# wwyuan2023/VITS

Measured on AMD Instinct MI355X. Metric: 22.05 kHz audio samples/sec/GPU (infer RTF) + train utt/sec at 1/2/4/8 MI355X, higher is better.
Workload: dtype fp32; 1 GPU; SynthesizerTrn.infer_p2 batch=16 Tx=100 Ty=500 (configs/base.json, 16 kHz, hop 192) per GPU; global_batch=16, seq_len=500, parallelism=single GPU, graph=False

## Files before the change

vits_amd/csrc/resblock_f32p.hip:

```cpp
#include "conv1d_impl.h"

namespace {

using vits_conv::fast_sigmoid;
using vits_conv::fast_tanh;
using vits_conv::split3_bf16x4;

constexpr int RP_GROUP = 3;
struct RpGroup {
  vits_resblock_pair_desc d[RP_GROUP];
  int n;
  int batch;
};

typedef __bf16 bf16x8 __attribute__((ext_vector_type(8)));
typedef __bf16 bf16x4 __attribute__((ext_vector_type(4)));
typedef __bf16 bf16x2 __attribute__((ext_vector_type(2)));
typedef float f32x4v __attribute__((ext_vector_type(4)));

template <int MODE>
struct RpT {
  typedef float xt;
  typedef __bf16 lt;
  static constexpr int NPL = 3;
};
template <>
struct RpT<1> {
  typedef __bf16 xt;
  typedef __bf16 lt;
  static constexpr int NPL = 1;
};
template <>
struct RpT<2> {
  typedef _Float16 xt;
  typedef _Float16 lt;
  static constexpr int NPL = 1;
};
__host__ __device__ constexpr int rp_npl(int mode) { return mode == 0 ? 3 : 1; }

__host__ __device__ constexpr int rp_ng(int C) { return C <= 64 ? 256 : 128; }
__host__ __device__ constexpr int rp_threads(int C) { return C == 256 ? 512 : 256; }
__host__ __device__ constexpr int rp_kc(int C, int mode = 0) {
  return C == 256 ? 64 : 16;
}
__host__ __device__ inline int rp_xcols(int NG, int k, int dil) {
  return ((NG + (k - 1) * dil + 3 + 3) >> 2) << 2;
}
__host__ __device__ inline int rp_lds_bytes(int C, int k, int dil, int mode = 0) {
  const int NG = rp_ng(C), npl = rp_npl(mode);
  const int xs = 2 * npl * rp_xcols(NG, k, dil) * (rp_kc(C, mode) + 4);
  const int gsz = npl * (NG + 16) * (C / 2 + 8);
  return 4 * 2 * C + 2 * (xs > gsz ? xs : gsz) + 64;
}
__host__ __device__ constexpr int rp_occ(int C, int) { return C == 256 ? 1 : 2; }

template <int C, int MODE = 0>
__global__ __launch_bounds__(rp_threads(C), rp_occ(C, MODE)) void resblock_f32p_kernel(
    const RpGroup G) {
  typedef typename RpT<MODE>::xt xt;
  typedef typename RpT<MODE>::lt lt;
  constexpr int NPL = RpT<MODE>::NPL;
  typedef lt lt8 __attribute__((ext_vector_type(8)));
  typedef lt lt4 __attribute__((ext_vector_type(4)));
  typedef lt lt2 __attribute__((ext_vector_type(2)));
  typedef xt xt4 __attribute__((ext_vector_type(4)));
  constexpr int H = C / 2;
  constexpr int NT = rp_threads(C);
  constexpr int WAVES_M = C >= 64 ? C / 64 : 1;
  constexpr int WAVES_N = NT / 64 / WAVES_M;
  constexpr int NG = 64 * WAVES_N;
  static_assert(NG == rp_ng(C), "tile columns");
  constexpr int TM = C >= 64 ? 2 : 1, TN = 2;
  constexpr int KC = rp_kc(C, MODE);
  constexpr int KCP = KC + 4;
  constexpr int GP = H + 8;
  constexpr int GPL = (NG + 16) * GP;
  constexpr int S1 = C / 16, S2 = H / 16;
  constexpr int NU = ((KC / 4) * ((NG + 102) / 4) + NT - 1) / NT;
  typedef lt8 av_t;
  constexpr int NB = NPL == 3 ? TN : 1;

  const int gi = (int)blockIdx.z / G.batch;
  const int b = (int)blockIdx.z - gi * G.batch;
  const vits_resblock_pair_desc& p = G.d[gi];
  const int Tn = p.t_len;
  const int L = p.lengths ? min(Tn, (int)p.lengths[b]) : Tn;
  const int k = p.k;
  const int dil = p.dil;
  const int BN = NG - (k - 1);
  const int n0 = blockIdx.x * BN;
  if (n0 >= Tn) return;
  if (p.lengths && p.len_skip > 0 && n0 >= L + p.len_skip) return;

  extern __shared__ float smem[];
  float* const erow = smem;
  lt* const reg = reinterpret_cast<lt*>(smem + 2 * C);

  const int tid = threadIdx.x;
  const int lane = tid & 63;
  const int wid = tid >> 6;
  const int wn = (wid % WAVES_N) * 64;
  const int wm = (wid / WAVES_N) * 64;
  const int l32 = lane & 31;
  const int lhi = lane >> 5;
  const int p1 = (k - 1) * dil / 2;
  const int p2 = (k - 1) / 2;

  {
    const float* cond = p.cond ? p.cond + (int64_t)b * p.cond_bstride : nullptr;
    for (int r = tid; r < 2 * C; r += NT) {
      float e = 0.f;
      if (r < C) {
        const int idx = (r & 1) ? H + (r >> 1) : (r >> 1);
        if (p.b1) e = p.b1[idx];
        if (cond) e += cond[idx];
      } else if (p.b2) {
        e = p.b2[r - C];
      }
      erow[r] = e;
    }
  }

  f32x16 acc[TM][TN];
#pragma unroll
  for (int i = 0; i < TM; ++i)
#pragma unroll
    for (int j = 0; j < TN; ++j)
#pragma unroll
      for (int r = 0; r < 16; ++r) acc[i][j][r] = 0.f;

  auto mma = [&](av_t (*a)[TM], const av_t* bh, const av_t* bm, const av_t* bl) {
#pragma unroll
    for (int mi = 0; mi < TM; ++mi)
#pragma unroll
      for (int ni = 0; ni < TN; ++ni) {
        f32x16 c = acc[mi][ni];
        if constexpr (MODE == 0) {
          c = __builtin_amdgcn_mfma_f32_32x32x16_bf16(a[0][mi], bl[ni], c, 0, 0, 0);
          c = __builtin_amdgcn_mfma_f32_32x32x16_bf16(a[2][mi], bh[ni], c, 0, 0, 0);
          c = __builtin_amdgcn_mfma_f32_32x32x16_bf16(a[1][mi], bm[ni], c, 0, 0, 0);
          c = __builtin_amdgcn_mfma_f32_32x32x16_bf16(a[0][mi], bm[ni], c, 0, 0, 0);
          c = __builtin_amdgcn_mfma_f32_32x32x16_bf16(a[1][mi], bh[ni], c, 0, 0, 0);
          c = __builtin_amdgcn_mfma_f32_32x32x16_bf16(a[0][mi], bh[ni], c, 0, 0, 0);
        } else if constexpr (MODE == 1) {
          c = __builtin_amdgcn_mfma_f32_32x32x16_bf16(a[0][mi], bh[ni], c, 0, 0, 0);
        } else {
          c = __builtin_amdgcn_mfma_f32_32x32x16_f16(a[0][mi], bh[ni], c, 0, 0, 0);
        }
        acc[mi][ni] = c;
      }
  };
  auto loadA = [&](const lt* wl, int64_t wstep, int m_pad, int s, int total,
                   av_t (*a)[TM]) {
    const lt* wp = wl + (int64_t)(s < total ? s : total - 1) * wstep;
#pragma unroll
    for (int q = 0; q < NPL; ++q)
#pragma unroll
      for (int mi = 0; mi < TM; ++mi)
        a[q][mi] = *reinterpret_cast<const av_t*>(wp + ((int64_t)q * m_pad + mi * 32) * 8);
  };

  av_t a0[NPL][TM], a1[NPL][TM];
  av_t bh0[TN], bm0[NB], bl0[NB], bh1[TN], bm1[NB], bl1[NB];

  const xt* xb = reinterpret_cast<const xt*>(p.x) + (int64_t)b * p.x_bstride;
  {
    const int tw0 = n0 - p2 - p1;
    const int xstart = tw0 & ~3;
    const int xsh = tw0 - xstart;
    const int xcols = rp_xcols(NG, k, dil);
    const int nunits = (KC / 4) * (xcols >> 2);
    const int xpl = xcols * KCP;
    lt* const xbuf0 = reg;
    lt* const xbuf1 = reg + NPL * xpl;
    const float slope = p.in_slope;
    xt4 xr[NU][4];
    int xoff[NU];
    bool xok[NU];
#pragma unroll
    for (int q = 0; q < NU; ++q) {
      const int u = tid + NT * q;
      const int tt = xstart + 4 * (u / (KC / 4));
      xok[q] = u < nunits && tt >= 0 && tt < Tn;
      xoff[q] = xok[q] ? 4 * (u % (KC / 4)) * p.x_cstride + tt : 0;
    }
    auto gload = [&](int ch) {
      const xt* base = xb + (int64_t)ch * KC * p.x_cstride;
#pragma unroll
      for (int q = 0; q < NU; ++q) {
        if (q * NT < nunits) {
#pragma unroll
          for (int i = 0; i < 4; ++i) {
            const xt* src = xok[q] ? base + xoff[q] + i * p.x_cstride : xb;
            xr[q][i] = *reinterpret_cast<const xt4*>(src);
          }
        }
      }
    };
    auto lstore = [&](lt* xs) {
#pragma unroll
      for (int q = 0; q < NU; ++q) {
        const int u = tid + NT * q;
        if (q * NT < nunits && u < nunits) {
          f32x4v v[4];
#pragma unroll
          for (int i = 0; i < 4; ++i)
#pragma unroll
            for (int e = 0; e < 4; ++e) {
              float t = (float)xr[q][i][e];
              t = t < 0.f ? t * slope : t;
              v[i][e] = xok[q] ? t : 0.f;
            }
          lt* xh = xs + 4 * (u / (KC / 4)) * KCP + 4 * (u % (KC / 4));
#pragma unroll
          for (int e = 0; e < 4; ++e) {
            const f32x4v w = {v[0][e], v[1][e], v[2][e], v[3][e]};
            if constexpr (NPL == 3) {
              bf16x4 h4, m4, l4;
              split3_bf16x4(w, h4, m4, l4);
              *reinterpret_cast<bf16x4*>(xh + e * KCP) = h4;
              *reinterpret_cast<bf16x4*>(xh + xpl + e * KCP) = m4;
              *reinterpret_cast<bf16x4*>(xh + 2 * xpl + e * KCP) = l4;
            } else {
              lt4 w4;
#pragma unroll
              for (int i = 0; i < 4; ++i) w4[i] = (lt)w[i];
              *reinterpret_cast<lt4*>(xh + e * KCP) = w4;
            }
          }
        }
      }
    };
    auto loadB = [&](const lt* xs, int j, int g, av_t* bh, av_t* bm, av_t* bl) {
      const int P4 = xpl / 4;
#pragma unroll
      for (int ni = 0; ni < TN; ++ni) {
        const lt4* xp = reinterpret_cast<const lt4*>(
            xs + (wn + ni * 32 + l32 + j * dil + xsh) * KCP + 16 * g + 8 * lhi);
        bh[ni] = __builtin_shufflevector(xp[0], xp[1], 0, 1, 2, 3, 4, 5, 6, 7);
        if constexpr (NPL == 3) {
          bm[ni] = __builtin_shufflevector(xp[P4], xp[P4 + 1], 0, 1, 2, 3, 4, 5, 6, 7);
          bl[ni] = __builtin_shufflevector(xp[2 * P4], xp[2 * P4 + 1], 0, 1, 2, 3, 4, 5, 6, 7);
        }
      }
    };
    const lt* wl = reinterpret_cast<const lt*>(p.w1) +
                   ((int64_t)(lhi * NPL) * p.m_pad1 + wm + l32) * 8;
    const int64_t wstep = (int64_t)16 * NPL * p.m_pad1;
    const int total = S1 * k;
    const int nst = (KC / 16) * k;
    loadA(wl, wstep, p.m_pad1, 0, total, a0);
    gload(0);
    lstore(xbuf0);
    __syncthreads();
    for (int ch = 0; ch < C / KC; ++ch) {
      const bool more = ch + 1 < C / KC;
      if (more) gload(ch + 1);
      const lt* xs = (ch & 1) ? xbuf1 : xbuf0;
      const int s0 = ch * nst;
      int j = 0, g = 0;
      auto next = [&]() {
        if (++j == k) {
          j = 0;
          ++g;
        }
      };
      loadB(xs, 0, 0, bh0, bm0, bl0);
      int st = 0;
      for (; st + 2 <= nst; st += 2) {
        next();
        loadA(wl, wstep, p.m_pad1, s0 + st + 1, total, a1);
        loadB(xs, j, g, bh1, bm1, bl1);
        __builtin_amdgcn_sched_barrier(0);
        mma(a0, bh0, bm0, bl0);
        __builtin_amdgcn_sched_barrier(0);
        next();
        loadA(wl, wstep, p.m_pad1, s0 + st + 2, total, a0);
        if (st + 2 < nst) loadB(xs, j, g, bh0, bm0, bl0);
        __builtin_amdgcn_sched_barrier(0);
        mma(a1, bh1, bm1, bl1);
        __builtin_amdgcn_sched_barrier(0);
      }
      if (st < nst) {
        loadA(wl, wstep, p.m_pad1, s0 + nst, total, a1);
        __builtin_amdgcn_sched_barrier(0);
        mma(a0, bh0, bm0, bl0);
#pragma unroll
        for (int q = 0; q < NPL; ++q)
#pragma unroll
          for (int mi = 0; mi < TM; ++mi) a0[q][mi] = a1[q][mi];
      }
      if (more) lstore((ch & 1) ? xbuf0 : xbuf1);
      __syncthreads();
    }
  }

  lt* const gs = reg;
#pragma unroll
  for (int mi = 0; mi < TM; ++mi) {
#pragma unroll
    for (int ni = 0; ni < TN; ++ni) {
      const int col = wn + ni * 32 + l32;
      const int t = n0 - p2 + col;
      const bool in = t >= 0 && t < L;
#pragma unroll
      for (int r = 0; r < 16; r += 4) {
        const int row = wm + mi * 32 + 4 * lhi + 8 * (r >> 2);
        const float g0 = fast_tanh(acc[mi][ni][r] + erow[row]) *
                         fast_sigmoid(acc[mi][ni][r + 1] + erow[row + 1]);
        const float g1 = fast_tanh(acc[mi][ni][r + 2] + erow[row + 2]) *
                         fast_sigmoid(acc[mi][ni][r + 3] + erow[row + 3]);
        lt* gp = gs + col * GP + (row >> 1);
        if constexpr (NPL == 3) {
          const f32x4v w = {in ? g0 : 0.f, in ? g1 : 0.f, 0.f, 0.f};
          bf16x4 h4, m4, l4;
          split3_bf16x4(w, h4, m4, l4);
          *reinterpret_cast<bf16x2*>(gp) = __builtin_shufflevector(h4, h4, 0, 1);
          *reinterpret_cast<bf16x2*>(gp + GPL) = __builtin_shufflevector(m4, m4, 0, 1);
          *reinterpret_cast<bf16x2*>(gp + 2 * GPL) = __builtin_shufflevector(l4, l4, 0, 1);
        } else {
          lt2 v2;
          v2[0] = (lt)(in ? g0 : 0.f);
          v2[1] = (lt)(in ? g1 : 0.f);
          *reinterpret_cast<lt2*>(gp) = v2;
        }
      }
#pragma unroll
      for (int r = 0; r < 16; ++r) acc[mi][ni][r] = 0.f;
    }
  }
  for (int i = tid; i < NPL * 16 * H; i += NT) {
    const int pl = i / (16 * H);
    const int e = i - pl * 16 * H;
    gs[pl * GPL + (NG + e / H) * GP + e % H] = (lt)0.f;
  }
  __syncthreads();

  {
    const lt* wl = reinterpret_cast<const lt*>(p.w2) +
                   ((int64_t)(lhi * NPL) * p.m_pad2 + wm + l32) * 8;
    const int64_t wstep = (int64_t)16 * NPL * p.m_pad2;
    const int total = S2 * k;
    const lt* gl = gs + (wn + l32) * GP + 8 * lhi;
    int j = 0, g = 0;
    auto loadB = [&](av_t* bh, av_t* bm, av_t* bl) {
      const lt* x = gl + j * GP + 16 * g;
#pragma unroll
      for (int ni = 0; ni < TN; ++ni) {
        bh[ni] = *reinterpret_cast<const av_t*>(x + ni * 32 * GP);
        if constexpr (NPL == 3) {
          bm[ni] = *reinterpret_cast<const av_t*>(x + ni * 32 * GP + GPL);
          bl[ni] = *reinterpret_cast<const av_t*>(x + ni * 32 * GP + 2 * GPL);
        }
      }
      if (++j == k) {
        j = 0;
        ++g;
      }
    };
    loadA(wl, wstep, p.m_pad2, 0, total, a0);
    loadB(bh0, bm0, bl0);
    int s = 0;
    for (; s + 2 <= total; s += 2) {
      loadA(wl, wstep, p.m_pad2, s + 1, total, a1);
      loadB(bh1, bm1, bl1);
      __builtin_amdgcn_sched_barrier(0);
      mma(a0, bh0, bm0, bl0);
      __builtin_amdgcn_sched_barrier(0);
      loadA(wl, wstep, p.m_pad2, s + 2, total, a0);
      if (s + 2 < total) loadB(bh0, bm0, bl0);
      __builtin_amdgcn_sched_barrier(0);
      mma(a1, bh1, bm1, bl1);
      __builtin_amdgcn_sched_barrier(0);
    }
    if (s < total) mma(a0, bh0, bm0, bl0);
  }

  xt* const yb = reinterpret_cast<xt*>(p.y) + (int64_t)b * p.y_bstride;
#pragma unroll
  for (int mi = 0; mi < TM; ++mi) {
#pragma unroll
    for (int ni = 0; ni < TN; ++ni) {
      const int col = wn + ni * 32 + l32;
      const int t = n0 + col;
      const bool st = col < BN && t < Tn;
      const int tc = st ? t : 0;
      float rv[16], yo[16];
#pragma unroll
      for (int r = 0; r < 16; ++r) {
        const int row = wm + mi * 32 + 4 * lhi + (r & 3) + 8 * (r >> 2);
        rv[r] = (float)xb[(int64_t)row * p.x_cstride + tc];
      }
      if (p.accumulate) {
#pragma unroll
        for (int r = 0; r < 16; ++r) {
          const int row = wm + mi * 32 + 4 * lhi + (r & 3) + 8 * (r >> 2);
          yo[r] = (float)yb[(int64_t)row * p.y_cstride + tc];
        }
      }
      if (st) {
#pragma unroll
        for (int r = 0; r < 16; ++r) {
          const int row = wm + mi * 32 + 4 * lhi + (r & 3) + 8 * (r >> 2);
          const float v = acc[mi][ni][r] + erow[C + row];
          float o = rv[r] + v;
          if (p.accumulate) o = yo[r] + o;
          if (p.post_div != 1.0f) o = o / p.post_div;
          yb[(int64_t)row * p.y_cstride + t] = (xt)(t < L ? o : 0.f);
        }
      }
    }
  }
}

template <int C, int MODE = 0>
int rp_launch(const RpGroup& g, hipStream_t s) {
  int lds = 0, gx = 0;
  for (int i = 0; i < g.n; ++i) {
    const vits_resblock_pair_desc& d = g.d[i];
    const int l = rp_lds_bytes(C, d.k, d.dil, MODE);
    if (l > lds) lds = l;
    const int BN = rp_ng(C) - (d.k - 1);
    const int x = (d.t_len + BN - 1) / BN;
    if (x > gx) gx = x;
  }
  if (lds > 160 * 1024) return VITS_E_UNSUP;
  hipLaunchKernelGGL((resblock_f32p_kernel<C, MODE>), dim3(gx, 1, g.n * g.batch),
                     dim3(rp_threads(C)), lds, s, g);
  return vits_launch_status();
}

int rp_check(const vits_resblock_pair_desc& d, int mode = 0) {
  VITS_CHECK_ARG(d.x && d.w1 && d.w2 && d.y);
  VITS_CHECK_ARG(reinterpret_cast<const void*>(d.y) != reinterpret_cast<const void*>(d.x));
  VITS_CHECK_SHAPE(d.channels == 32 || d.channels == 64 || d.channels == 128 ||
                   d.channels == 256);
  VITS_CHECK_SHAPE(d.k >= 1 && d.k <= 15 && (d.k & 1) == 1 && d.dil >= 1 && d.t_len > 0);
  VITS_CHECK_SHAPE((d.k - 1) * d.dil <= 96);
  VITS_CHECK_SHAPE(d.m_pad1 >= d.channels && d.m_pad2 >= d.channels && (d.m_pad1 & 3) == 0 &&
                   (d.m_pad2 & 3) == 0);
  VITS_CHECK_SHAPE(d.cin_pad1 >= d.channels && d.cin_pad2 >= d.channels / 2);
  VITS_CHECK_SHAPE((d.t_len & 3) == 0 && (d.x_cstride & 3) == 0 && (d.x_bstride & 3) == 0 &&
                   d.x_cstride >= d.t_len && d.y_cstride >= d.t_len &&
                   (reinterpret_cast<uintptr_t>(d.x) & (mode ? 7 : 15)) == 0);
  VITS_CHECK_SHAPE((int64_t)d.channels * d.x_cstride < (1LL << 31));
  VITS_CHECK_SHAPE((reinterpret_cast<uintptr_t>(d.w1) & 15) == 0 &&
                   (reinterpret_cast<uintptr_t>(d.w2) & 15) == 0);
  return VITS_OK;
}

}

int vits_rp16_256(const vits_resblock_pair_desc* d, int n, int batch, int wdtype,
                  hipStream_t s) {
  if (!d || n < 1 || n > RP_GROUP || batch < 1) return VITS_E_ARG;
  if (wdtype != VITS_WDT_BF16 && wdtype != VITS_WDT_F16) return VITS_E_ARG;
  const int mode = wdtype == VITS_WDT_BF16 ? 1 : 2;
  RpGroup g;
  g.n = n;
  g.batch = batch;
  for (int i = 0; i < n; ++i) {
    const int rc = rp_check(d[i], mode);
    if (rc) return rc;
    if (d[i].channels != d[0].channels) return VITS_E_SHAPE;
    g.d[i] = d[i];
  }
  if (d[0].channels != 256) return VITS_E_SHAPE;
  return mode == 1 ? rp_launch<256, 1>(g, s) : rp_launch<256, 2>(g, s);
}

extern "C" int vits_resblock_pair_f32p_forward(const vits_resblock_pair_desc* d, int n, int batch,
                                               void* stream) {
  if (!d || n < 1 || n > RP_GROUP || batch < 1) return VITS_E_ARG;
  RpGroup g;
  g.n = n;
  g.batch = batch;
  for (int i = 0; i < n; ++i) {
    const int rc = rp_check(d[i]);
    if (rc) return rc;
    if (d[i].channels != d[0].channels) return VITS_E_SHAPE;
    g.d[i] = d[i];
  }
  hipStream_t s = as_stream(stream);
  int rc;
  if (d[0].channels == 32)
    rc = rp_launch<32>(g, s);
  else if (d[0].channels == 64)
    rc = rp_launch<64>(g, s);
  else if (d[0].channels == 128)
    rc = rp_launch<128>(g, s);
  else
    rc = rp_launch<256>(g, s);
  return count_ok(rc, VITS_CNT_RESBLOCK);
}
```

Baseline: 78.75 million output samples/s.

## Make resblock pair kernel persistent with cross-tile prefetch and pipelined epilogue

Replaces the 3D grid of one tile per workgroup with a persistent grid sized to CU count (1 or 2 per CU), where each workgroup walks a flattened tile list ordered by descending kernel size. The first input chunk of the next tile is loaded during the current tile's second conv and epilogue, and the epilogue's residual/accumulate loads are split into double-buffered halves. The aim is to hide global-load latency across tiles, avoid tail imbalance and reuse bias rows when the group and batch are unchanged. In exchange it adds register pressure from the extra prefetch buffers, a serial tile-walking loop, and an env var cap on workgroup count.

```diff
diff --git a/vits_amd/csrc/resblock_f32p.hip b/vits_amd/csrc/resblock_f32p.hip
--- a/vits_amd/csrc/resblock_f32p.hip
+++ b/vits_amd/csrc/resblock_f32p.hip
@@ -1,3 +1,6 @@
+#include <atomic>
+#include <cstdlib>
+
 #include "conv1d_impl.h"
 
 namespace {
@@ -11,6 +14,9 @@
   vits_resblock_pair_desc d[RP_GROUP];
   int n;
   int batch;
+  int order[RP_GROUP];
+  int nx[RP_GROUP];
+  int start[RP_GROUP + 1];
 };
 
 typedef __bf16 bf16x8 __attribute__((ext_vector_type(8)));
@@ -80,54 +86,45 @@
   typedef lt8 av_t;
   constexpr int NB = NPL == 3 ? TN : 1;
 
-  const int gi = (int)blockIdx.z / G.batch;
-  const int b = (int)blockIdx.z - gi * G.batch;
-  const vits_resblock_pair_desc& p = G.d[gi];
-  const int Tn = p.t_len;
-  const int L = p.lengths ? min(Tn, (int)p.lengths[b]) : Tn;
-  const int k = p.k;
-  const int dil = p.dil;
-  const int BN = NG - (k - 1);
-  const int n0 = blockIdx.x * BN;
-  if (n0 >= Tn) return;
-  if (p.lengths && p.len_skip > 0 && n0 >= L + p.len_skip) return;
+  const int ntiles = G.start[G.n];
+  const int nwg = (int)gridDim.x;
+  auto seek = [&](int t, int& gi, int& b, int& n0, int& L) {
+    for (; t < ntiles; t += nwg) {
+      int m = 0;
+      while (m + 1 < G.n && t >= G.start[m + 1]) ++m;
+      gi = G.order[m];
+      const vits_resblock_pair_desc& q = G.d[gi];
+      const int loc = t - G.start[m];
+      b = loc / G.nx[m];
+      n0 = (loc - b * G.nx[m]) * (NG - (q.k - 1));
+      L = q.lengths ? min(q.t_len, __builtin_amdgcn_readfirstlane((int)q.lengths[b])) : q.t_len;
+      if (n0 >= q.t_len) continue;
+      if (q.lengths && q.len_skip > 0 && n0 >= L + q.len_skip) continue;
+      break;
+    }
+    return t;
+  };
+  int gi, b, n0, L;
+  int tile = seek((int)blockIdx.x, gi, b, n0, L);
+  if (tile >= ntiles) return;
 
   extern __shared__ float smem[];
   float* const erow = smem;
   lt* const reg = reinterpret_cast<lt*>(smem + 2 * C);
 
-  const int tid = threadIdx.x;
-  const int lane = tid & 63;
-  const int wid = tid >> 6;
-  const int wn = (wid % WAVES_N) * 64;
-  const int wm = (wid / WAVES_N) * 64;
-  const int l32 = lane & 31;
-  const int lhi = lane >> 5;
-  const int p1 = (k - 1) * dil / 2;
-  const int p2 = (k - 1) / 2;
-
-  {
-    const float* cond = p.cond ? p.cond + (int64_t)b * p.cond_bstride : nullptr;
-    for (int r = tid; r < 2 * C; r += NT) {
-      float e = 0.f;
-      if (r < C) {
-        const int idx = (r & 1) ? H + (r >> 1) : (r >> 1);
-        if (p.b1) e = p.b1[idx];
-        if (cond) e += cond[idx];
-      } else if (p.b2) {
-        e = p.b2[r - C];
-      }
-      erow[r] = e;
-    }
-  }
+  int tid = threadIdx.x;
+  int lane, wid, wn, wm, l32, lhi;
+  auto ids = [&]() {
+    lane = tid & 63;
+    wid = tid >> 6;
+    wn = (wid % WAVES_N) * 64;
+    wm = (wid / WAVES_N) * 64;
+    l32 = lane & 31;
+    lhi = lane >> 5;
+  };
+  ids();
 
   f32x16 acc[TM][TN];
-#pragma unroll
-  for (int i = 0; i < TM; ++i)
-#pragma unroll
-    for (int j = 0; j < TN; ++j)
-#pragma unroll
-      for (int r = 0; r < 16; ++r) acc[i][j][r] = 0.f;
 
   auto mma = [&](av_t (*a)[TM], const av_t* bh, const av_t* bm, const av_t* bl) {
 #pragma unroll
@@ -163,40 +160,89 @@
   av_t a0[NPL][TM], a1[NPL][TM];
   av_t bh0[TN], bm0[NB], bl0[NB], bh1[TN], bm1[NB], bl1[NB];
 
-  const xt* xb = reinterpret_cast<const xt*>(p.x) + (int64_t)b * p.x_bstride;
+  const xt* xb;
+  int xcs;
+  int xsh;
+  int nunits;
+  int xpl;
+  float slope;
+  xt4 xr[NU][4];
+  int xoff[NU];
+  bool xok[NU];
+  auto stage = [&](int gi_, int b_, int n0_) {
+    const vits_resblock_pair_desc& q = G.d[gi_];
+    xb = reinterpret_cast<const xt*>(q.x) + (int64_t)b_ * q.x_bstride;
+    xcs = q.x_cstride;
+    slope = q.in_slope;
+    const int tw0 = n0_ - (q.k - 1) / 2 - (q.k - 1) * q.dil / 2;
+    const int xstart = tw0 & ~3;
+    xsh = tw0 - xstart;
+    const int xcols = rp_xcols(NG, q.k, q.dil);
+    nunits = (KC / 4) * (xcols >> 2);
+    xpl = xcols * KCP;
+#pragma unroll
+    for (int u_ = 0; u_ < NU; ++u_) {
+      const int u = tid + NT * u_;
+      const int tt = xstart + 4 * (u / (KC / 4));
+      xok[u_] = u < nunits && tt >= 0 && tt < q.t_len;
+      xoff[u_] = xok[u_] ? 4 * (u % (KC / 4)) * xcs + tt : 0;
+    }
+  };
+  auto gload = [&](int ch) {
+    const xt* base = xb + (int64_t)ch * KC * xcs;
+#pragma unroll
+    for (int q = 0; q < NU; ++q) {
+      if (q * NT < nunits) {
+#pragma unroll
+        for (int i = 0; i < 4; ++i) {
+          const xt* src = xok[q] ? base + xoff[q] + i * xcs : xb;
+          xr[q][i] = *reinterpret_cast<const xt4*>(src);
+        }
+      }
+    }
+  };
+  stage(gi, b, n0);
+  gload(0);
+  int egi = -1, eb = -1;
+
+  for (;;) {
+  asm volatile("" : "+v"(tid));
+  ids();
+  const vits_resblock_pair_desc& p = G.d[gi];
+  const int Tn = p.t_len;
+  const int k = p.k;
+  const int dil = p.dil;
+  const int BN = NG - (k - 1);
+  const int p2 = (k - 1) / 2;
+  const xt* const xbr = xb;
+
+  if (gi != egi || b != eb) {
+    const float* cond = p.cond ? p.cond + (int64_t)b * p.cond_bstride : nullptr;
+    for (int r = tid; r < 2 * C; r += NT) {
+      float e = 0.f;
+      if (r < C) {
+        const int idx = (r & 1) ? H + (r >> 1) : (r >> 1);
+        if (p.b1) e = p.b1[idx];
+        if (cond) e += cond[idx];
+      } else if (p.b2) {
+        e = p.b2[r - C];
+      }
+      erow[r] = e;
+    }
+    egi = gi;
+    eb = b;
+  }
+
+#pragma unroll
+  for (int i = 0; i < TM; ++i)
+#pragma unroll
+    for (int j = 0; j < TN; ++j)
+#pragma unroll
+      for (int r = 0; r < 16; ++r) acc[i][j][r] = 0.f;
+
   {
-    const int tw0 = n0 - p2 - p1;
-    const int xstart = tw0 & ~3;
-    const int xsh = tw0 - xstart;
-    const int xcols = rp_xcols(NG, k, dil);
-    const int nunits = (KC / 4) * (xcols >> 2);
-    const int xpl = xcols * KCP;
     lt* const xbuf0 = reg;
     lt* const xbuf1 = reg + NPL * xpl;
-    const float slope = p.in_slope;
-    xt4 xr[NU][4];
-    int xoff[NU];
-    bool xok[NU];
-#pragma unroll
-    for (int q = 0; q < NU; ++q) {
-      const int u = tid + NT * q;
-      const int tt = xstart + 4 * (u / (KC / 4));
-      xok[q] = u < nunits && tt >= 0 && tt < Tn;
-      xoff[q] = xok[q] ? 4 * (u % (KC / 4)) * p.x_cstride + tt : 0;
-    }
-    auto gload = [&](int ch) {
-      const xt* base = xb + (int64_t)ch * KC * p.x_cstride;
-#pragma unroll
-      for (int q = 0; q < NU; ++q) {
-        if (q * NT < nunits) {
-#pragma unroll
-          for (int i = 0; i < 4; ++i) {
-            const xt* src = xok[q] ? base + xoff[q] + i * p.x_cstride : xb;
-            xr[q][i] = *reinterpret_cast<const xt4*>(src);
-          }
-        }
-      }
-    };
     auto lstore = [&](lt* xs) {
 #pragma unroll
       for (int q = 0; q < NU; ++q) {
@@ -250,7 +296,6 @@
     const int total = S1 * k;
     const int nst = (KC / 16) * k;
     loadA(wl, wstep, p.m_pad1, 0, total, a0);
-    gload(0);
     lstore(xbuf0);
     __syncthreads();
     for (int ch = 0; ch < C / KC; ++ch) {
@@ -295,6 +340,13 @@
     }
   }
 
+  int ngi, nb, nn0, nL;
+  const int ntile = seek(tile + nwg, ngi, nb, nn0, nL);
+  if (ntile < ntiles) {
+    stage(ngi, nb, nn0);
+    gload(0);
+  }
+
   lt* const gs = reg;
 #pragma unroll
   for (int mi = 0; mi < TM; ++mi) {
@@ -336,6 +388,30 @@
   }
   __syncthreads();
 
+  xt* const yb = reinterpret_cast<xt*>(p.y) + (int64_t)b * p.y_bstride;
+  constexpr int ER = 8;
+  constexpr int EU = TM * TN * 16 / ER;
+  float rv[2][ER], yo[2][ER];
+  auto epi_load = [&](int u, float* rv_, float* yo_) {
+    const int si = u / (16 / ER), r0 = u % (16 / ER) * ER;
+    const int mi = si / TN, ni = si % TN;
+    const int col = wn + ni * 32 + l32;
+    const int t = n0 + col;
+    const int tc = col < BN && t < Tn ? t : 0;
+#pragma unroll
+    for (int r = r0; r < r0 + ER; ++r) {
+      const int row = wm + mi * 32 + 4 * lhi + (r & 3) + 8 * (r >> 2);
+      rv_[r - r0] = (float)xbr[(int64_t)row * p.x_cstride + tc];
+    }
+    if (p.accumulate) {
+#pragma unroll
+      for (int r = r0; r < r0 + ER; ++r) {
+        const int row = wm + mi * 32 + 4 * lhi + (r & 3) + 8 * (r >> 2);
+        yo_[r - r0] = (float)yb[(int64_t)row * p.y_cstride + tc];
+      }
+    }
+  };
+
   {
     const lt* wl = reinterpret_cast<const lt*>(p.w2) +
                    ((int64_t)(lhi * NPL) * p.m_pad2 + wm + l32) * 8;
@@ -376,57 +452,96 @@
     if (s < total) mma(a0, bh0, bm0, bl0);
   }
 
-  xt* const yb = reinterpret_cast<xt*>(p.y) + (int64_t)b * p.y_bstride;
-#pragma unroll
-  for (int mi = 0; mi < TM; ++mi) {
-#pragma unroll
-    for (int ni = 0; ni < TN; ++ni) {
-      const int col = wn + ni * 32 + l32;
-      const int t = n0 + col;
-      const bool st = col < BN && t < Tn;
-      const int tc = st ? t : 0;
-      float rv[16], yo[16];
+  epi_load(0, rv[0], yo[0]);
+#pragma unroll
+  for (int mi = 0; mi < TM; ++mi)
+#pragma unroll
+    for (int ni = 0; ni < TN; ++ni)
 #pragma unroll
       for (int r = 0; r < 16; ++r) {
         const int row = wm + mi * 32 + 4 * lhi + (r & 3) + 8 * (r >> 2);
-        rv[r] = (float)xb[(int64_t)row * p.x_cstride + tc];
-      }
-      if (p.accumulate) {
-#pragma unroll
-        for (int r = 0; r < 16; ++r) {
-          const int row = wm + mi * 32 + 4 * lhi + (r & 3) + 8 * (r >> 2);
-          yo[r] = (float)yb[(int64_t)row * p.y_cstride + tc];
-        }
-      }
-      if (st) {
-#pragma unroll
-        for (int r = 0; r < 16; ++r) {
-          const int row = wm + mi * 32 + 4 * lhi + (r & 3) + 8 * (r >> 2);
-          const float v = acc[mi][ni][r] + erow[C + row];
-          float o = rv[r] + v;
-          if (p.accumulate) o = yo[r] + o;
-          if (p.post_div != 1.0f) o = o / p.post_div;
-          yb[(int64_t)row * p.y_cstride + t] = (xt)(t < L ? o : 0.f);
-        }
-      }
-    }
-  }
+        acc[mi][ni][r] = acc[mi][ni][r] + erow[C + row];
+      }
+  __syncthreads();
+
+#pragma unroll
+  for (int u = 0; u < EU; ++u) {
+    const int si = u / (16 / ER), r0 = u % (16 / ER) * ER;
+    const int mi = si / TN, ni = si % TN;
+    if (u + 1 < EU) epi_load(u + 1, rv[(u + 1) & 1], yo[(u + 1) & 1]);
+    const int col = wn + ni * 32 + l32;
+    const int t = n0 + col;
+    if (col < BN && t < Tn) {
+#pragma unroll
+      for (int r = r0; r < r0 + ER; ++r) {
+        const int row = wm + mi * 32 + 4 * lhi + (r & 3) + 8 * (r >> 2);
+        const float v = acc[mi][ni][r];
+        float o = rv[u & 1][r - r0] + v;
+        if (p.accumulate) o = yo[u & 1][r - r0] + o;
+        if (p.post_div != 1.0f) o = o / p.post_div;
+        yb[(int64_t)row * p.y_cstride + t] = (xt)(t < L ? o : 0.f);
+      }
+    }
+  }
+
+  if (ntile >= ntiles) break;
+  tile = ntile;
+  gi = ngi;
+  b = nb;
+  n0 = nn0;
+  L = nL;
+  }
+}
+
+int rp_cus() {
+  constexpr int MAXDEV = 64;
+  static std::atomic<int> cus[MAXDEV];
+  int dev = 0;
+  if (hipGetDevice(&dev) != hipSuccess || dev < 0 || dev >= MAXDEV) dev = 0;
+  int n = cus[dev].load(std::memory_order_relaxed);
+  if (n <= 0) {
+    if (hipDeviceGetAttribute(&n, hipDeviceAttributeMultiprocessorCount, dev) != hipSuccess ||
+        n <= 0)
+      n = 256;
+    cus[dev].store(n, std::memory_order_relaxed);
+  }
+  return n;
+}
+
+int rp_wg_cap() {
+  const char* e = getenv("VITS_RP_MAX_WG");
+  const int v = e ? atoi(e) : 0;
+  return v > 0 ? v : 0;
 }
 
 template <int C, int MODE = 0>
-int rp_launch(const RpGroup& g, hipStream_t s) {
-  int lds = 0, gx = 0;
+int rp_launch(RpGroup& g, hipStream_t s) {
+  int lds = 0;
   for (int i = 0; i < g.n; ++i) {
     const vits_resblock_pair_desc& d = g.d[i];
     const int l = rp_lds_bytes(C, d.k, d.dil, MODE);
     if (l > lds) lds = l;
+    int m = i;
+    for (; m > 0 && g.d[g.order[m - 1]].k < d.k; --m) g.order[m] = g.order[m - 1];
+    g.order[m] = i;
+  }
+  if (lds > 160 * 1024) return VITS_E_UNSUP;
+  int64_t tiles = 0;
+  for (int m = 0; m < g.n; ++m) {
+    const vits_resblock_pair_desc& d = g.d[g.order[m]];
     const int BN = rp_ng(C) - (d.k - 1);
-    const int x = (d.t_len + BN - 1) / BN;
-    if (x > gx) gx = x;
-  }
-  if (lds > 160 * 1024) return VITS_E_UNSUP;
-  hipLaunchKernelGGL((resblock_f32p_kernel<C, MODE>), dim3(gx, 1, g.n * g.batch),
-                     dim3(rp_threads(C)), lds, s, g);
+    g.nx[m] = (d.t_len + BN - 1) / BN;
+    g.start[m] = (int)tiles;
+    tiles += (int64_t)g.nx[m] * g.batch;
+    if (tiles >= (1LL << 30)) return VITS_E_SHAPE;
+  }
+  g.start[g.n] = (int)tiles;
+  int64_t wgs = (int64_t)rp_cus() * (C == 256 ? 1 : 2);
+  const int cap = rp_wg_cap();
+  if (cap && cap < wgs) wgs = cap;
+  if (tiles < wgs) wgs = tiles;
+  hipLaunchKernelGGL((resblock_f32p_kernel<C, MODE>), dim3((unsigned)wgs), dim3(rp_threads(C)),
+                     lds, s, g);
   return vits_launch_status();
 }
 
```

After: 78.43 million output samples/s. No clear change (-0.4%).
